# vsois/hanabi-agents

Hardware: AMD Instinct MI355X
Metric: env_steps_per_sec (higher is better)
Workload: dtype u8 env/encoder + bfloat16 Q-net GEMM (fp32 accumulate, fp32 master weights)

## Files before the change

hanabi-agents_amd/csrc/actor_fused.hip:

```cpp
#include <hip/hip_runtime.h>
#include <hip/hip_bf16.h>
#include <hip/hip_fp16.h>

#include <cstdint>
#include <type_traits>

#include "../../include/hanabi_hip.h"
#include "common.hpp"
#include "env_kernel.hpp"

using hb::fail;

namespace {

typedef __bf16 bf16x8 __attribute__((ext_vector_type(8)));
typedef _Float16 f16x8 __attribute__((ext_vector_type(8)));
typedef float f32x4 __attribute__((ext_vector_type(4)));

constexpr int FM = 128;
constexpr int FH = 512;
constexpr int FNT = 512;
constexpr int FK = 51;
constexpr int S2 = FH / 32;
constexpr int LUT_BYTES = 65536;
// ... 391 lines not shown
      if (ea < A && row < a.m) {
        const float* f = reinterpret_cast<const float*>(lds + H_BYTES) + (4 * g) * FM + rr;
        const float m0 = f[0], m1 = f[FM], m2 = f[2 * FM], m3 = f[3 * FM];
        const float M = fmaxf(fmaxf(m0, m1), fmaxf(m2, m3));
        const float e0 = exp2_fast(m0 - M), e1 = exp2_fast(m1 - M), e2 = exp2_fast(m2 - M), e3 = exp2_fast(m3 - M);
        const float* fs = f + 8 * FM;
        const float* ft = f + 16 * FM;
        const float S = fs[0] * e0 + fs[FM] * e1 + fs[2 * FM] * e2 + fs[3 * FM] * e3;
        const float T = ft[0] * e0 + ft[FM] * e1 + ft[2 * FM] * e2 + ft[3 * FM] * e3;
        a.q[row * A + ea] = T * __builtin_amdgcn_rcpf(S) * (1.0f / FK);
      }
    }
    if (p + 1 < n_pass) __syncthreads();
    if (p < 2) HB_FSTAMP(9 + 3 * p);
  }
  if (a.legal) {
    asm volatile("s_waitcnt vmcnt(0)" ::: "memory");
    __syncthreads();
    if (tid < FM && row0 + tid < a.m) {
      const long long g = row0 + tid;
      const unsigned long long gid = static_cast<unsigned long long>(a.first_gid + g);
      uint32_t rnd[4];
      hb::philox4x32_10(static_cast<uint32_t>(a.draw), static_cast<uint32_t>(a.draw >> 32), static_cast<uint32_t>(gid),
                        static_cast<uint32_t>(gid >> 32), static_cast<uint32_t>(a.seed), static_cast<uint32_t>(a.seed >> 32), rnd);
      const float* qr = a.q + g * A;
      const int8_t* lr = a.legal + g * A;
      float best = -INFINITY;
      unsigned long long legal_mask = 0, ties = 0;
      for (int i = 0; i < A; ++i) {
        const float v = __hip_atomic_load(qr + i, __ATOMIC_RELAXED, __HIP_MEMORY_SCOPE_AGENT);
        if (lr[i] != 0) {
          legal_mask |= 1ull << i;
          if (v > best) { best = v; ties = 1ull << i; }
          else if (v == best) ties |= 1ull << i;
        }
      }
      const float u = static_cast<float>(rnd[0] >> 8) * (1.0f / 16777216.0f);
      unsigned long long pool = (u < a.epsilon) ? legal_mask : ties;
      if (pool == 0) pool = legal_mask;
      int pick = 0;
      const int c = __popcll(pool);
      if (c > 0) {
        int k = static_cast<int>(__umulhi(rnd[1], static_cast<uint32_t>(c)));
        while (k-- > 0) pool &= pool - 1;
        pick = __ffsll(static_cast<long long>(pool)) - 1;
      }
      a.actions[g] = pick;
      if constexpr (!std::is_void_v<K>) reinterpret_cast<int*>(lds + H_BYTES)[tid] = pick;
    }
  }
  if constexpr (!std::is_void_v<K>) {
    constexpr int ENV_WORDS = hb::env_lds_words<K, EG>();
    static_assert((FM / EG) * ENV_WORDS * 4 <= H_BYTES && FM / EG <= FNT / 64, "env tail: the LDS slices must fit in H");
    __syncthreads();
    if (wave < FM / EG) {
#if defined(__HIP_DEVICE_COMPILE__)
      typedef const __attribute__((address_space(4))) unsigned char KargByte;
      typedef const __attribute__((address_space(4))) hb::EnvArgs KargEnv;
      auto kargs = __builtin_amdgcn_kernarg_segment_ptr();
      asm volatile("" : "+s"(kargs));
      constexpr size_t ENV_OFF = (sizeof(FusedArgs) + alignof(hb::EnvArgs) - 1) / alignof(hb::EnvArgs) * alignof(hb::EnvArgs);
      KargEnv& env = *(KargEnv*)((KargByte*)kargs + ENV_OFF);
#else
      const hb::EnvArgs env{};
#endif
      const long long g0 = row0 + EG * wave;
      const int uid = lane < EG ? reinterpret_cast<const int*>(lds + H_BYTES)[EG * wave + lane] : 0;
      hb::env_wave_step<K, EG>(env, g0, lane, reinterpret_cast<uint32_t*>(lds) + wave * ENV_WORDS, uid, g0 / EG);
    }
  }
  HB_FSTAMP_REAL(15);
}

template <bool F16>
__global__ __launch_bounds__(FNT) void actor_fused_kernel(const FusedArgs a) {
  actor_fused_body<F16, void, 16>(a);
}

template <bool F16, class K, int EG>
__global__ __launch_bounds__(FNT) void actor_env_fused_kernel(const FusedArgs a, const hb::EnvArgs env) {
  (void)env;
  actor_fused_body<F16, K, EG>(a);
}

template <bool F16>
__global__ __launch_bounds__(FNT) void actor_fused_grouped_kernel(const FusedArgs a, const hb_fused_tile* __restrict__ tiles) {
  const hb_fused_tile& t = tiles[blockIdx.x];
  if (!t.active) return;
  FusedArgs b = a;
  b.w1f = static_cast<const uint4*>(t.w1f); b.b1 = t.b1f; b.w2f = static_cast<const uint4*>(t.w2f); b.b2 = t.b2f;
  b.support = t.support;
  b.first_gid = t.first_game_id - static_cast<long long>(blockIdx.x) * FM;
  actor_fused_body<F16, void, 16>(b);
}

struct PackArgs {
  const __hip_bfloat16* w1; int w1_ld;
  const __hip_bfloat16* b1;
  const __hip_bfloat16* w2; int w2_ld;
  const __hip_bfloat16* b2;
  int obs_len, s1, n_actions, n_pass;
  uint4* w1f; float* b1f; uint4* w2f; float* b2f;
  int chunks1, chunks2;
  int f16;
  uint16_t* w1t; int w1t_ld;
  uint16_t* w2t; int w2t_ld;
};
__device__ __forceinline__ float bias_to_float(const __hip_bfloat16* b, int i, int f16) {
  return f16 ? __half2float(reinterpret_cast<const __half*>(b)[i]) : __bfloat162float(b[i]);
}
__host__ __device__ __forceinline__ int fused_logit(int col, int n_actions, int n_pass) {
  const int slot = col >> 6, c = col & 63, n = c >> 4, q = (c >> 2) & 3, j = c & 3;
  const int r16 = 4 * n + j;
  const int full_cap = 8 * n_pass;
  int action, atom;
  if (r16 < 12 || (r16 == 12 && q < 3)) {
    action = slot < full_cap ? slot : n_actions;
    if (action >= n_actions) return -1;
    atom = r16 < 12 ? 4 * r16 + q : 48 + q;
  } else {
    const int p = slot >> 3, w = slot & 7, f = w & 3;
// ... 280 lines not shown
```

hanabi-agents_amd/csrc/env_api.hip:

```cpp
#include <hip/hip_runtime.h>

#include <cstdarg>
#include <cstdio>
#include <cstdlib>
#include <cstring>
#include <new>
#include <string>
#include <vector>

#include "../../include/hanabi_hip.h"
#include "common.hpp"
#include "env_kernel.hpp"

namespace hb {
const EnvVariant* variants_full(int* n);
const EnvVariant* variants_small(int* n);
const EnvVariant* variants_vsmall(int* n);

thread_local std::string g_error;
int fail(int code, const char* fmt, ...) {
  char buf[512];
  va_list ap;
  va_start(ap, fmt);
  vsnprintf(buf, sizeof buf, fmt, ap);
  va_end(ap);
  g_error = buf;
  return code;
}

const EnvVariant* find_variant(const hb_config* c) {
  const EnvVariant* (*tables[])(int*) = {variants_full, variants_small, variants_vsmall};
  for (auto get : tables) {
    int n = 0;
    const EnvVariant* v = get(&n);
    for (int i = 0; i < n; ++i)
      if (v[i].P == c->players && v[i].C == c->colors && v[i].R == c->ranks && v[i].H == c->hand_size &&
          v[i].INFO == c->max_info && v[i].LIFE == c->max_life)
        return &v[i];
  }
  return nullptr;
}

static int copies_of(const hb_config* c, int r) { return r == 0 ? 3 : (r == c->ranks - 1 ? 1 : 2); }
static int deck_of(const hb_config* c) {
  int per = 0;
  for (int r = 0; r < c->ranks; ++r) per += copies_of(c, r);
  return per * c->colors;
}
}

struct hb_env {
  hb_config cfg;
  const hb::EnvVariant* var;
  long long n;
  unsigned long long seed;
  long long first_gid;
  uint32_t* state;
  unsigned long long* illegal;
  long long stat_slots;
  uint8_t* next_deck;
  uint8_t* refill;
  const uint8_t* decks;
  int gpw;
  int device;
  hipEvent_t ev_start, ev_stop;
  hipStream_t side;
  hipEvent_t ev_step_done, ev_refill_done;
  bool refill_in_flight;
  bool async_refill;
  int refill_period, since_refill;
  uint16_t* perms;
  uint8_t* shuf_mask;
  bool shuffled;
};

using hb::fail;

template <int C>
__global__ void color_perms_draw_kernel(const uint32_t* __restrict__ state, int sw, const uint8_t* __restrict__ mask, long long n, int P,
                                        unsigned long long seed, long long first_gid, uint16_t* __restrict__ perms) {
  const long long g = static_cast<long long>(blockIdx.x) * blockDim.x + threadIdx.x;
  if (g >= n) return;
  const uint32_t episode = state[g * sw + 6], m = mask[g];
  uint32_t e[hb::PERM_SLOTS / 2] = {0u, 0u, 0u, 0u};
  for (int p = 0; p < P; ++p) {
    const uint32_t sg = ((m >> p) & 1u) ? hb::draw_perm<C>(seed, static_cast<unsigned long long>(first_gid + g), episode, p)
                                        : hb::identity_perm(C);
    e[p >> 1] |= sg << (16 * (p & 1));
  }
  reinterpret_cast<uint4*>(perms)[g] = make_uint4(e[0], e[1], e[2], e[3]);
}

__global__ void color_perms_export_kernel(const uint16_t* __restrict__ perms, long long n, int P, int C, uint8_t* __restrict__ out) {
  const long long i = static_cast<long long>(blockIdx.x) * blockDim.x + threadIdx.x;
  if (i >= n * P * C) return;
  const long long g = i / (P * C);
  const int r = static_cast<int>(i - g * P * C), p = r / C, c = r - p * C;
  out[i] = static_cast<uint8_t>(perms ? (perms[g * hb::PERM_SLOTS + p] >> (3 * c)) & 7u : static_cast<uint32_t>(c));
}

__global__ void color_perms_import_kernel(const uint8_t* __restrict__ in, long long n, int P, int C, uint16_t* __restrict__ perms) {
  const long long g = static_cast<long long>(blockIdx.x) * blockDim.x + threadIdx.x;
  if (g >= n) return;
  uint32_t e[hb::PERM_SLOTS / 2] = {0u, 0u, 0u, 0u};
  for (int p = 0; p < P; ++p) {
    uint32_t sg = 0;
    for (int c = 0; c < C; ++c) sg |= static_cast<uint32_t>(in[(g * P + p) * C + c] & 7u) << (3 * c);
    e[p >> 1] |= sg << (16 * (p & 1));
  }
  reinterpret_cast<uint4*>(perms)[g] = make_uint4(e[0], e[1], e[2], e[3]);
}

static int draw_color_perms(hb_env* e, void* stream) {
  if (!e->shuffled) return HB_OK;
  const unsigned blocks = static_cast<unsigned>((e->n + 255) / 256);
  const hipStream_t st = static_cast<hipStream_t>(stream);
  const int P = e->cfg.players, sw = e->var->state_words;
  switch (e->cfg.colors) {
    case 1: hipLaunchKernelGGL(color_perms_draw_kernel<1>, dim3(blocks), dim3(256), 0, st, e->state, sw, e->shuf_mask, e->n, P, e->seed, e->first_gid, e->perms); break;
    case 2: hipLaunchKernelGGL(color_perms_draw_kernel<2>, dim3(blocks), dim3(256), 0, st, e->state, sw, e->shuf_mask, e->n, P, e->seed, e->first_gid, e->perms); break;
    case 3: hipLaunchKernelGGL(color_perms_draw_kernel<3>, dim3(blocks), dim3(256), 0, st, e->state, sw, e->shuf_mask, e->n, P, e->seed, e->first_gid, e->perms); break;
    case 4: hipLaunchKernelGGL(color_perms_draw_kernel<4>, dim3(blocks), dim3(256), 0, st, e->state, sw, e->shuf_mask, e->n, P, e->seed, e->first_gid, e->perms); break;
    default: hipLaunchKernelGGL(color_perms_draw_kernel<5>, dim3(blocks), dim3(256), 0, st, e->state, sw, e->shuf_mask, e->n, P, e->seed, e->first_gid, e->perms); break;
// ... 9 lines not shown

int hb_config_validate(const hb_config* c) {
  if (!c) return fail(HB_ERR_INVALID, "null config");
  if (c->players < 2 || c->players > 5) return fail(HB_ERR_INVALID, "players must be 2..5 (got %d)", c->players);
  if (c->colors < 1 || c->colors > 5) return fail(HB_ERR_INVALID, "colors must be 1..5 (got %d)", c->colors);
  if (c->ranks < 1 || c->ranks > 5) return fail(HB_ERR_INVALID, "ranks must be 1..5 (got %d)", c->ranks);
  if (c->hand_size < 1 || c->hand_size > 5) return fail(HB_ERR_INVALID, "hand_size must be 1..5 (got %d)", c->hand_size);
  if (c->max_info < 1 || c->max_info > 15) return fail(HB_ERR_INVALID, "max_info must be 1..15");
  if (c->max_life < 1 || c->max_life > 7) return fail(HB_ERR_INVALID, "max_life must be 1..7");
  if (c->players * c->hand_size > hb::deck_of(c)) return fail(HB_ERR_INVALID, "deck too small for the hands");
  return HB_OK;
}
int hb_num_actions(const hb_config* c) { return 2 * c->hand_size + (c->players - 1) * (c->colors + c->ranks); }
int hb_deck_size(const hb_config* c) { return hb::deck_of(c); }
int hb_obs_len(const hb_config* c) {
  const int bits = c->colors * c->ranks, P = c->players, H = c->hand_size, D = hb::deck_of(c);
  return (P - 1) * H * bits + P + (D - P * H + bits + c->max_info + c->max_life) + D +
         (P + 4 + P + c->colors + c->ranks + H + H + bits + 2) + P * H * (bits + c->colors + c->ranks);
}
int hb_state_words(const hb_config* c) { return c->players <= 3 ? 32 : 48; }
int hb_obs_words(const hb_config* c) { return (hb_obs_len(c) + 31) / 32; }

int hb_env_create(const hb_config* cfg, int64_t n_games, uint64_t seed, int64_t first_game_id, hb_env** out) {
  if (!out) return fail(HB_ERR_INVALID, "null out");
  *out = nullptr;
  if (int rc = hb_config_validate(cfg)) return rc;
  if (n_games <= 0) return fail(HB_ERR_INVALID, "n_games must be positive");
  const hb::EnvVariant* var = hb::find_variant(cfg);
  if (!var)
    return fail(HB_ERR_INVALID,
                "no compiled kernel for players=%d colors=%d ranks=%d hand=%d info=%d life=%d "
                "(built: Hanabi-Full / -Small / -Very-Small, 2..5 players)",
                cfg->players, cfg->colors, cfg->ranks, cfg->hand_size, cfg->max_info, cfg->max_life);
  if (var->obs_len != hb_obs_len(cfg) || var->n_actions != hb_num_actions(cfg) || var->deck != hb_deck_size(cfg))
    return fail(HB_ERR_INVALID, "internal: kernel sizes disagree with host formulas");
  int ndev = 0;
  if (hipGetDeviceCount(&ndev) != hipSuccess || ndev <= 0) return fail(HB_ERR_NO_DEVICE, "no HIP device available");
  hb_env* e = new (std::nothrow) hb_env();
  if (!e) return fail(HB_ERR_NOMEM, "out of host memory");
  e->cfg = *cfg;
  e->var = var;
  e->n = n_games;
  e->seed = seed;
  e->first_gid = first_game_id;
  e->decks = nullptr;
  e->gpw = 0;
  e->ev_start = e->ev_stop = nullptr;
  e->side = nullptr;
  e->ev_step_done = e->ev_refill_done = nullptr;
  e->refill_in_flight = false;
  e->async_refill = false;
  e->refill_period = cfg->max_life < 3 ? cfg->max_life : 3;
  e->since_refill = 0;
  e->perms = nullptr;
  e->shuf_mask = nullptr;
  e->shuffled = false;
  HB_HIP_OR(hipGetDevice(&e->device), delete e);
  const size_t bytes = static_cast<size_t>(n_games) * var->state_words * 4;
  HB_HIP_OR(hipMalloc(reinterpret_cast<void**>(&e->state), bytes), delete e);
  e->stat_slots = n_games / 8 + 8;
  HB_HIP_OR(hipMalloc(reinterpret_cast<void**>(&e->illegal), 8 + 16 * e->stat_slots), { (void)hipFree(e->state); delete e; });
  HB_HIP_OR(hipMemset(e->state, 0, bytes), { hb_env_destroy(e); });
  HB_HIP_OR(hipMemset(e->illegal, 0, 8 + 16 * e->stat_slots), { hb_env_destroy(e); });
  HB_HIP_OR(hipMalloc(reinterpret_cast<void**>(&e->next_deck), static_cast<size_t>(n_games) * hb::NEXT_DECK_BYTES), { hb_env_destroy(e); });
  HB_HIP_OR(hipMalloc(reinterpret_cast<void**>(&e->refill), static_cast<size_t>(n_games)), { hb_env_destroy(e); });
  HB_HIP_OR(hipMemset(e->next_deck, 0, static_cast<size_t>(n_games) * hb::NEXT_DECK_BYTES), { hb_env_destroy(e); });
  HB_HIP_OR(hipMemset(e->refill, 1, static_cast<size_t>(n_games)), { hb_env_destroy(e); });
  HB_HIP_OR(hipStreamCreateWithFlags(&e->side, hipStreamNonBlocking), { hb_env_destroy(e); });
  HB_HIP_OR(hipEventCreateWithFlags(&e->ev_step_done, hipEventDisableTiming), { hb_env_destroy(e); });
  HB_HIP_OR(hipEventCreateWithFlags(&e->ev_refill_done, hipEventDisableTiming), { hb_env_destroy(e); });
  *out = e;
  return HB_OK;
}

int hb_env_destroy(hb_env* e) {
  if (!e) return HB_OK;
  if (e->state) (void)hipFree(e->state);
  if (e->illegal) (void)hipFree(e->illegal);
  if (e->next_deck) (void)hipFree(e->next_deck);
  if (e->refill) (void)hipFree(e->refill);
  if (e->perms) (void)hipFree(e->perms);
  if (e->shuf_mask) (void)hipFree(e->shuf_mask);
  if (e->side) { (void)hipStreamSynchronize(e->side); (void)hipStreamDestroy(e->side); }
  if (e->ev_step_done) (void)hipEventDestroy(e->ev_step_done);
  if (e->ev_refill_done) (void)hipEventDestroy(e->ev_refill_done);
  delete e;
  return HB_OK;
}

int64_t hb_env_num_games(const hb_env* e) { return e ? e->n : 0; }

int hb_env_set_decks(hb_env* e, const uint8_t* decks_dev) {
  if (!e) return fail(HB_ERR_INVALID, "null env");
  e->decks = decks_dev;
  e->refill_in_flight = false;
  HB_HIP(hipDeviceSynchronize());
  HB_HIP(hipMemset(e->refill, 1, static_cast<size_t>(e->n)));
  return HB_OK;
}

int hb_env_set_games_per_wave(hb_env* e, int32_t g) {
  if (!e) return fail(HB_ERR_INVALID, "null env");
  if (g != 0 && g != 8 && g != 16 && g != 32 && g != 64)
    return fail(HB_ERR_INVALID, "games per wave must be 0 (automatic), 8, 16, 32 or 64");
  e->gpw = g;
  return HB_OK;
}

int hb_env_set_profile_events(hb_env* e, void* start_event, void* stop_event) {
  if (!e) return fail(HB_ERR_INVALID, "null env");
  if ((start_event == nullptr) != (stop_event == nullptr)) return fail(HB_ERR_INVALID, "pass both events or neither");
  e->ev_start = static_cast<hipEvent_t>(start_event);
  e->ev_stop = static_cast<hipEvent_t>(stop_event);
  return HB_OK;
}

static void fill_common(hb_env* e, hb::EnvArgs& a) {
  a.state = e->state;
  a.decks = e->decks;
  a.next_deck = e->next_deck;
  a.refill = e->refill;
  a.illegal = e->illegal;
  a.stats = e->illegal + 1;
  a.n = e->n;
  a.seed = e->seed;
  a.first_gid = e->first_gid;
  a.flags = e->cfg.flags;
}

static int join_refill(hb_env* e, void* stream) {
  if (e->refill_in_flight) {
    HB_HIP(hipStreamWaitEvent(static_cast<hipStream_t>(stream), e->ev_refill_done, 0));
    e->refill_in_flight = false;
  }
  return HB_OK;
}

static int refill(hb_env* e, void* stream) {
  e->since_refill = 0;
  hb::EnvArgs a{};
  fill_common(e, a);
  e->var->refill(a, static_cast<hipStream_t>(stream));
  HB_HIP(hipGetLastError());
  return HB_OK;
}

static int refill_async(hb_env* e, void* stream) {
  if (++e->since_refill < e->refill_period) return HB_OK;
  if (!e->async_refill) return refill(e, stream);
  HB_HIP(hipEventRecord(e->ev_step_done, static_cast<hipStream_t>(stream)));
  HB_HIP(hipStreamWaitEvent(e->side, e->ev_step_done, 0));
  if (int rc = refill(e, e->side)) return rc;
  HB_HIP(hipEventRecord(e->ev_refill_done, e->side));
  e->refill_in_flight = true;
  return HB_OK;
}

static void prepare(hb_env* e, hb::EnvArgs& a) {
  a.state = e->state;
  a.decks = e->decks;
  a.next_deck = e->next_deck;
  a.refill = e->refill;
  a.illegal = e->illegal;
  a.stats = e->illegal + 1;
  a.n = e->n;
  a.seed = e->seed;
  a.first_gid = e->first_gid;
  a.flags = e->cfg.flags;
  a.ev_start = e->ev_start;
  a.ev_stop = e->ev_stop;
  a.perms = e->shuffled ? e->perms : nullptr;
  a.shuf_mask = e->shuffled ? e->shuf_mask : nullptr;
}

static int launch(hb_env* e, hb::EnvArgs& a, void* stream) {
  prepare(e, a);
  const int gpw = e->gpw ? e->gpw : ((a.obs_bits && !a.obs && e->n >= 32768) ? 32 : 16);
  const hb::EnvVariant& v = *e->var;
  hb::LaunchFn fn = e->shuffled ? (gpw == 8 ? v.s8 : (gpw == 16 ? v.s16 : (gpw == 32 ? v.s32 : v.s64)))
                                : (gpw == 8 ? v.g8 : (gpw == 16 ? v.g16 : (gpw == 32 ? v.g32 : v.g64)));
  fn(a, static_cast<hipStream_t>(stream));
  HB_HIP(hipGetLastError());
  return HB_OK;
}

static int check_out(const void* obs, const void* legal) {
  if (!obs || !legal) return fail(HB_ERR_INVALID, "obs_dev and legal_dev are required");
  if ((reinterpret_cast<uintptr_t>(obs) & 15) || (reinterpret_cast<uintptr_t>(legal) & 15))
    return fail(HB_ERR_ALIGN, "obs_dev / legal_dev must be 16-byte aligned");
  return HB_OK;
}
static int check_out_packed(const void* bits, const void* obs, const void* legal) {
// ... 160 lines not shown
  if (!e) return fail(HB_ERR_INVALID, "null env");
  if (!q_dev || !sel_legal_dev || !actions_out_dev) return fail(HB_ERR_INVALID, "q_dev, sel_legal_dev and actions_out_dev are required");
  if ((reinterpret_cast<uintptr_t>(q_dev) & 15) || (reinterpret_cast<uintptr_t>(sel_legal_dev) & 3))
    return fail(HB_ERR_ALIGN, "q_dev must be 16-byte and sel_legal_dev 4-byte aligned");
  if (e->var->n_actions > 64) return fail(HB_ERR_INVALID, "the fused selection handles at most 64 actions");
  if (int rc = check_out_packed(obs_bits_dev, obs_dev, legal_dev)) return rc;
  hb::EnvArgs a{};
  a.mode = hb::MODE_STEP;
  a.sel_q = q_dev;
  a.sel_legal = sel_legal_dev;
  a.sel_actions = actions_out_dev;
  a.sel_eps = epsilon;
  a.sel_seed = seed;
  a.sel_draw = draw;
  a.sel_first_gid = first_game_id;
  a.obs = obs_dev;
  a.obs_bits = obs_bits_dev;
  a.legal = legal_dev;
  a.reward = reward_dev;
  a.terminal = terminal_dev;
  a.agent_reward = agent_reward_dev;
  a.agent_step_type = agent_step_type_dev;
  a.score = score_dev;
  if (int rc = join_refill(e, stream)) return rc;
  if (int rc = launch(e, a, stream)) return rc;
  return refill_async(e, stream);
}

int hb_actor_fused_act_step(hb_env* e, const uint32_t* obs_bits_dev, const int8_t* legal_dev, int64_t n_rows, int32_t obs_len,
                            const void* w1f_dev, const float* b1f_dev, const void* w2f_dev, const float* b2f_dev, const float* support_dev,
                            int32_t hidden, int32_t n_actions, int32_t n_atoms, float* q_dev, float epsilon, uint64_t seed, uint64_t draw,
                            int64_t first_game_id, int32_t* actions_dev, int32_t dtype, uint32_t* obs_bits_out_dev, int8_t* legal_out_dev,
                            float* reward_dev, int8_t* terminal_dev, float* agent_reward_dev, int8_t* agent_step_type_dev,
                            int8_t* score_dev, void* stream) {
  if (!e) return fail(HB_ERR_INVALID, "null env");
  if (e->shuffled) return fail(HB_ERR_INVALID, "the fused policy + env kernel has no colour-permuted form: step a shuffled env with "
                                               "hb_env_step_packed or hb_env_step_select_packed");
  if (int rc = check_out_packed(obs_bits_out_dev, nullptr, legal_out_dev)) return rc;
  hb::EnvArgs a{};
  a.mode = hb::MODE_STEP;
  a.obs_bits = obs_bits_out_dev;
  a.legal = legal_out_dev;
  a.reward = reward_dev;
  a.terminal = terminal_dev;
  a.agent_reward = agent_reward_dev;
  a.agent_step_type = agent_step_type_dev;
  a.score = score_dev;
  prepare(e, a);
  if (int rc = join_refill(e, stream)) return rc;
  if (int rc = hb::actor_env_fused_launch(obs_bits_dev, legal_dev, n_rows, obs_len, w1f_dev, b1f_dev, w2f_dev, b2f_dev, support_dev, hidden,
                                          n_actions, n_atoms, q_dev, epsilon, seed, draw, first_game_id, actions_dev, dtype, a, *e->var,
                                          stream))
    return rc;
  return refill_async(e, stream);
}

int hb_actor_fused_step_supported(const hb_env* e) { return e && !e->shuffled && hb::actor_env_fused_supported(*e->var) ? 1 : 0; }

#ifdef HB_STAMPS
int hb_env_step_stamped(hb_env* e, const int32_t* actions_dev, int8_t* obs_dev, int8_t* legal_dev,
                        unsigned long long* stamps_dev, void* stream) {
  hb::EnvArgs a{};
  a.mode = hb::MODE_STEP;
  a.actions = actions_dev;
  a.obs = obs_dev;
  a.legal = legal_dev;
  a.stamps = stamps_dev;
  if (int rc = join_refill(e, stream)) return rc;
  if (int rc = launch(e, a, stream)) return rc;
  return refill_async(e, stream);
}
#endif

int hb_env_illegal_count(hb_env* e, int64_t* out) {
  if (!e || !out) return fail(HB_ERR_INVALID, "null argument");
  unsigned long long v = 0;
  HB_HIP(hipMemcpy(&v, e->illegal, 8, hipMemcpyDeviceToHost));
  *out = static_cast<int64_t>(v);
  return HB_OK;
}

int hb_env_stats(hb_env* e, int64_t* episodes, int64_t* score_sum) {
  if (!e || !episodes || !score_sum) return fail(HB_ERR_INVALID, "null argument");
  std::vector<unsigned long long> v(static_cast<size_t>(2 * e->stat_slots));
  HB_HIP(hipMemcpy(v.data(), e->illegal + 1, 16 * e->stat_slots, hipMemcpyDeviceToHost));
  unsigned long long ep = 0, sc = 0;
  for (long long i = 0; i < e->stat_slots; ++i) { ep += v[2 * i]; sc += v[2 * i + 1]; }
  *episodes = static_cast<int64_t>(ep);
  *score_sum = static_cast<int64_t>(sc);
  return HB_OK;
}

int hb_env_set_refill_period(hb_env* e, int32_t steps) {
  if (!e) return fail(HB_ERR_INVALID, "null env");
  if (steps < 1 || steps > e->cfg.max_life) return fail(HB_ERR_INVALID, "refill period must be 1..max_life (%d)", e->cfg.max_life);
  e->refill_period = steps;
  return HB_OK;
}

int hb_env_set_async_refill(hb_env* e, int32_t on) {
  if (!e) return fail(HB_ERR_INVALID, "null env");
  HB_HIP(hipDeviceSynchronize());
  e->refill_in_flight = false;
  e->async_refill = on != 0;
  return HB_OK;
}

// ... 77 lines not shown
```

hanabi-agents_amd/csrc/env_kernel.hpp:

```cpp
#pragma once
#include <hip/hip_runtime.h>
#include <hip/hip_ext.h>
#include <stdint.h>
#include <utility>

struct hb_config;

namespace hb {

enum { MODE_STEP = 0, MODE_OBSERVE = 1, MODE_RESET = 2 };
constexpr int NEXT_DECK_BYTES = 64;
enum { MV_PLAY = 0, MV_DISCARD = 1, MV_RCOLOR = 2, MV_RRANK = 3 };

struct EnvArgs {
  uint32_t* state;
  const int32_t* actions;
  const uint8_t* mask;
  const uint8_t* decks;
  uint8_t* next_deck;
  uint8_t* refill;
  int8_t* obs;
  uint32_t* obs_bits;
  int8_t* legal;
  float* reward;
// ... 356 lines not shown
      dv |= ((disc >> (c * K::CPC)) & ((1ull << K::CPC) - 1ull)) << (K::CPC * sig(c));
    });
    acc.template put64<K::DISC_OFF, K::D>(dv);
  } else {
    acc.template put64<K::DISC_OFF, K::D>(disc);
  }
  {
    const uint32_t valid = w2 & 1u;
    const int la_player = (w2 >> 1) & 7, la_type = (w2 >> 4) & 3, la_ci = (w2 >> 6) & 7, la_toff = (w2 >> 9) & 7;
    const int la_color_t = (w2 >> 12) & 7, la_rank = (w2 >> 15) & 7;
    const int la_color = SHUF ? sig(la_color_t) : la_color_t;
    const uint32_t la_scored = (w2 >> 18) & 1u, la_info = (w2 >> 19) & 1u, la_mask = (w2 >> 20) & 31u;
    int actor = la_player - o;
    if (actor < 0) actor += P;
    int target = actor + la_toff;
    if (target >= P) target -= P;
    const uint32_t reveal = valid & static_cast<uint32_t>(la_type >= MV_RCOLOR);
    const uint32_t cardmv = valid & static_cast<uint32_t>(la_type <= MV_DISCARD);
    const uint32_t is_rc = valid & static_cast<uint32_t>(la_type == MV_RCOLOR);
    const uint32_t is_rr = valid & static_cast<uint32_t>(la_type == MV_RRANK);
    const uint32_t is_play = valid & static_cast<uint32_t>(la_type == MV_PLAY);
    constexpr int o1 = K::LA_OFF, o2 = o1 + P, o3 = o2 + 4, o4 = o3 + P, o5 = o4 + C, o6 = o5 + R, o7 = o6 + H,
                  o8 = o7 + H, o9 = o8 + K::BITS;
    acc.template put<o1, P>(valid << actor);
    acc.template put<o2, 4>(valid << la_type);
    acc.template put<o3, P>(reveal << target);
    acc.template put<o4, C>(is_rc << la_color);
    acc.template put<o5, R>(is_rr << la_rank);
    acc.template put<o6, H>(reveal ? la_mask : 0u);
    acc.template put<o7, H>(cardmv << la_ci);
    acc.template put<o8, K::BITS>(cardmv << (la_color * R + la_rank));
    acc.template put<o9, 2>((is_play & la_scored) | ((is_play & la_info) << 1));
  }
  static_for<P>([&](auto REL) {
    constexpr int rel = decltype(REL)::value;
    int p = o + rel;
    if (p >= P) p -= P;
    const int n_p = hand_n(p);
    const uint64_t kn = (static_cast<uint64_t>(row[K::W_KNOW + 2 * p + 1]) << 32) | row[K::W_KNOW + 2 * p];
    static_for<H>([&](auto I) {
      constexpr int i = decltype(I)::value;
      const uint32_t k = static_cast<uint32_t>(kn >> (12 * i)) & 0xFFFu;
      const uint32_t cp = seen_colours<SHUF, C>(k & 31u, sg), rp = (k >> 5) & 31u;
      const uint32_t plaus = __umul24(spread_colors<C, R>(cp), rp);
      const uint32_t ch = (k >> 10) & 1u, rh = (k >> 11) & 1u;
      uint64_t v = plaus | (static_cast<uint64_t>(ch ? cp : 0u) << K::BITS) |
                   (static_cast<uint64_t>(rh ? rp : 0u) << (K::BITS + C));
      if (i >= n_p) v = 0;
      acc.template put64<K::KN_OFF + (rel * H + i) * K::KN_SLOT, K::KN_SLOT>(v);
    });
  });
}

template <class K, int G, bool SHUF = false>
__device__ __forceinline__ void env_wave_step(const EnvArgs& a, long long g0, int lane, uint32_t* const srow, int uid_in,
                                              long long wslot) {
  constexpr int P = K::P, C = K::C, R = K::R, H = K::H;
  constexpr int LPG = 1;
  uint32_t* const obits = srow + G * K::SWP;
  uint32_t* const lbits = obits + G * K::NWP;
  const long long left = a.n - g0;
  const int nvalid = left <= 0 ? 0 : (left < G ? static_cast<int>(left) : G);
  const int mode = a.mode;
  HB_STAMP_REAL(10);
  HB_STAMP(0);

  const bool active = lane < nvalid && lane < G;
  const long long gi = g0 + lane;
  bool mask_in = true;
  uint4 nd[4] = {make_uint4(0u, 0u, 0u, 0u), make_uint4(0u, 0u, 0u, 0u), make_uint4(0u, 0u, 0u, 0u), make_uint4(0u, 0u, 0u, 0u)};
  const uint4* const ndp = reinterpret_cast<const uint4*>(a.next_deck + gi * NEXT_DECK_BYTES);
  if (active) {
    if (mode == MODE_RESET && a.mask) mask_in = a.mask[gi] != 0;
    if (mode == MODE_RESET && mask_in) {
      nd[0] = ndp[0]; nd[1] = ndp[1]; nd[2] = ndp[2]; nd[3] = ndp[3];
    }
  }
  uint4 pm = make_uint4(0u, 0u, 0u, 0u);
  if constexpr (SHUF) {
    if (active) pm = reinterpret_cast<const uint4*>(a.perms)[gi];
  }

  {
    constexpr int Q = K::SW / 4;
    constexpr int ROUNDS = (G * Q + 63) / 64;
    const uint4* src = reinterpret_cast<const uint4*>(a.state + g0 * K::SW);
    uint4 v[ROUNDS];
#pragma unroll
    for (int r = 0; r < ROUNDS; ++r) {
      const int e = lane + 64 * r;
      v[r] = e < nvalid * Q ? src[e] : make_uint4(0u, 0u, 0u, 0u);
    }
#pragma unroll
    for (int r = 0; r < ROUNDS; ++r) {
      const int e = lane + 64 * r;
      if (e < nvalid * Q) {
        const int g = e / Q, q = e - g * Q;
        uint32_t* d = srow + g * K::SWP + 4 * q;
        d[0] = v[r].x; d[1] = v[r].y; d[2] = v[r].z; d[3] = v[r].w;
      }
    }
  }
  HB_STAMP(1);
  wave_sync();
  HB_STAMP(2);

  uint32_t* const row = srow + lane * K::SWP;
  uint32_t w0 = 0, w1 = 0, w2 = 0, w3 = 0, w6 = 0;
  uint64_t accw = 0, disc = 0;
// ... 111 lines not shown
        if (success) w1 += 1u << (3 * c_col);
        {
          const int dpos = (c_col * K::CPC + (c_rank ? 2 * c_rank + 1 : 0)) & 63;
          const uint32_t dmask = c_rank == 0 ? 7u : (c_rank == R - 1 ? 1u : 3u);
          const uint32_t dfield = static_cast<uint32_t>(disc >> dpos) & dmask;
          const uint32_t dnew = to_discard ? (((dfield << 1) | 1u) & dmask) : 0u;
          disc |= static_cast<uint64_t>(dnew) << dpos;
        }
        const int info2 = info + (card_move ? la_info : -1);
        const int life2 = life - (fail ? 1 : 0);
        const int deck2 = deck_size - ((card_move && draws) ? 1 : 0);
        const int turns2 = turns - (deck_size == 0 ? 1 : 0);
        const int la_color = card_move ? c_col : hcol, la_rank = card_move ? c_rank : hrank;
        w2 = 1u | (static_cast<uint32_t>(s) << 1) | (static_cast<uint32_t>(type) << 4) | (static_cast<uint32_t>(ci) << 6) |
             (static_cast<uint32_t>(toff) << 9) | (static_cast<uint32_t>(la_color) << 12) |
             (static_cast<uint32_t>(la_rank) << 15) | (static_cast<uint32_t>(success ? 1 : 0) << 18) |
             (static_cast<uint32_t>(card_move ? la_info : 0) << 19) | (match << 20);
        int cur = s + 1;
        if (cur >= P) cur = 0;
        w0 = static_cast<uint32_t>(deck2) | (static_cast<uint32_t>(info2) << 6) | (static_cast<uint32_t>(life2) << 10) |
             (static_cast<uint32_t>(cur) << 13) | (static_cast<uint32_t>(turns2 & 7) << 16) |
             (static_cast<uint32_t>((moves + 1) & 255) << 21);
        const int after = score_now();
        int status = 0;
        if (life2 < 1) status = 1;
        else if (after >= C * R) status = 2;
        else if (turns2 <= 0) status = 3;
        w0 |= static_cast<uint32_t>(status) << 19;
        int r = after - before;
        if ((a.flags & 4) && r < 0) r = 0;
        out_reward = static_cast<float>(r);
        out_term = status != 0;
#pragma unroll
        for (int q = 0; q < P; ++q) {
          const bool live = ((w3 >> q) & 1u) && !((w3 >> (5 + q)) & 1u);
          const int8_t v = static_cast<int8_t>(static_cast<int8_t>(accw >> (8 * q)) + (live ? r : 0));
          accw = (accw & ~(0xFFull << (8 * q))) | (static_cast<uint64_t>(static_cast<uint8_t>(v)) << (8 * q));
          if (live && out_term) w3 |= 1u << (5 + q);
        }
        if (out_term && (a.flags & 1)) {
          need_reset = true;
          reset_start = (a.flags & 2) ? cur : 0;
        }
      }
    }
    out_score = score_now();
  }

  HB_STAMP(3);
  if (active && need_reset) {
    const uint32_t* ndw = reinterpret_cast<const uint32_t*>(nd);
#pragma unroll
    for (int i = 0; i < 13; ++i) row[K::W_DECK + i] = ndw[i];
    a.refill[gi] = 1;
  }
  HB_STAMP(4);
  wave_sync();
  HB_STAMP(5);

  if (active) {
    if (need_reset) {
      const uint8_t* deckb = reinterpret_cast<const uint8_t*>(row + K::W_DECK);
      w0 = static_cast<uint32_t>(K::D - P * H) | (static_cast<uint32_t>(K::INFO) << 6) | (static_cast<uint32_t>(K::LIFE) << 10) |
           (static_cast<uint32_t>(reset_start) << 13) | (static_cast<uint32_t>(P) << 16);
      w1 = 0;
      w2 = 0;
      if (!keep_seats) { w3 = 0; accw = 0; }
      w6 += 1;
      disc = 0;
#pragma unroll
      for (int p = 0; p < P; ++p) {
        uint32_t hc = 0;
        uint64_t kn = 0;
#pragma unroll
        for (int i = 0; i < 5; ++i) {
          if (i < H) {
            hc |= static_cast<uint32_t>(deckb[p * H + i]) << (5 * i);
            kn |= static_cast<uint64_t>(K::ALL_PLAUSIBLE) << (12 * i);
          } else {
            hc |= 31u << (5 * i);
          }
        }
        row[K::W_HANDS + p] = hc;
        row[K::W_KNOW + 2 * p] = static_cast<uint32_t>(kn);
        row[K::W_KNOW + 2 * p + 1] = static_cast<uint32_t>(kn >> 32);
        w1 |= static_cast<uint32_t>(H) << (15 + 3 * p);
      }
      if constexpr (SHUF) {
        const uint32_t sm = a.shuf_mask[gi];
        uint32_t e[PERM_SLOTS / 2] = {0u, 0u, 0u, 0u};
#pragma unroll
        for (int p = 0; p < P; ++p) {
          const uint32_t sg = ((sm >> p) & 1u) ? draw_perm<C>(a.seed, static_cast<unsigned long long>(a.first_gid + gi), w6, p)
                                               : identity_perm(C);
          e[p >> 1] |= sg << (16 * (p & 1));
        }
        pm = make_uint4(e[0], e[1], e[2], e[3]);
        reinterpret_cast<uint4*>(a.perms)[gi] = pm;
      }
    }
    if (mode != MODE_OBSERVE) {
      row[0] = w0; row[1] = w1; row[2] = w2; row[3] = w3;
      row[4] = static_cast<uint32_t>(accw); row[5] = static_cast<uint32_t>(accw >> 32);
      row[6] = w6; row[7] = 0;
      row[8] = static_cast<uint32_t>(disc); row[9] = static_cast<uint32_t>(disc >> 32);
    }

// ... 18 lines not shown
      }
      const uint32_t pend = (w3 >> o) & 1u, tsin = (w3 >> (5 + o)) & 1u;
      if (a.agent_reward) a.agent_reward[gi] = pend ? static_cast<float>(static_cast<int8_t>(accw >> (8 * o))) : 0.f;
      if (a.agent_step_type) a.agent_step_type[gi] = static_cast<int8_t>(!pend ? 0 : (tsin ? 2 : 1));
      if (mode == MODE_STEP) {
        if (a.reward) a.reward[gi] = out_reward;
        if (a.terminal) a.terminal[gi] = static_cast<int8_t>(out_term);
        if (a.score) a.score[gi] = static_cast<int8_t>(out_score);
      }
    }
  }
  if (mode == MODE_STEP) {
    const unsigned long long bad = __ballot(illegal);
    if (bad && lane == 0) atomicAdd(a.illegal, static_cast<unsigned long long>(__popcll(bad)));
    const unsigned long long ended = __ballot(out_term != 0);
    if (ended) {
      int sc = out_term ? out_score : 0;
      for (int o = 32; o > 0; o >>= 1) sc += __shfl_xor(sc, o);
      if (lane == 0) {
        unsigned long long* slot = a.stats + 2 * wslot;
        atomicAdd(slot, static_cast<unsigned long long>(__popcll(ended)));
        atomicAdd(slot + 1, static_cast<unsigned long long>(sc));
      }
    }
  }
  HB_STAMP(6);
  wave_sync();
  HB_STAMP(7);

  if (mode != MODE_OBSERVE) {
    constexpr int Q = K::SW / 4;
    uint4* dst = reinterpret_cast<uint4*>(a.state + g0 * K::SW);
    for (int e = lane; e < nvalid * Q; e += 64) {
      const int g = e / Q, q = e - g * Q;
      const uint32_t* s = srow + g * K::SWP + 4 * q;
      uint4 v;
      v.x = s[0]; v.y = s[1]; v.z = s[2]; v.w = s[3];
      dst[e] = v;
    }
  }
  HB_STAMP(8);
  if (mode != MODE_RESET) {
    if (a.obs_bits) {
      uint32_t* dst = a.obs_bits + g0 * K::NW;
      for (int e = lane; e < nvalid * K::NW; e += 64) {
        const int g = e / K::NW, i = e - g * K::NW;
        dst[e] = obits[g * K::NWP + i];
      }
    }
    if (a.obs) expand_rows<K::OBS_LEN>(obits, K::NWP, nvalid, a.obs + g0 * K::OBS_LEN, lane);
    expand_rows<K::A>(lbits, K::LW, nvalid, a.legal + g0 * K::A, lane);
  }
  HB_STAMP(9);
  HB_STAMP_REAL(11);
}

template <class K, int G>
__global__ __launch_bounds__(256) void env_kernel(const EnvArgs a) {
  __shared__ uint32_t lds[4 * env_lds_words<K, G>()];
  const int lane = threadIdx.x & 63;
  const int wave = threadIdx.x >> 6;
  const long long wslot = static_cast<long long>(blockIdx.x) * 4 + wave;
  const long long g0 = wslot * G;
  int uid_in = 0;
  if (a.mode == MODE_STEP && lane < G && g0 + lane < a.n) uid_in = a.sel_q ? select_action<K::A>(a, g0 + lane) : a.actions[g0 + lane];
  env_wave_step<K, G>(a, g0, lane, lds + wave * env_lds_words<K, G>(), uid_in, wslot);
}

template <class K, int G>
__global__ __launch_bounds__(256) void env_kernel_shuf(const EnvArgs a) {
  __shared__ uint32_t lds[4 * env_lds_words<K, G>()];
  const int lane = threadIdx.x & 63;
  const int wave = threadIdx.x >> 6;
  const long long wslot = static_cast<long long>(blockIdx.x) * 4 + wave;
  const long long g0 = wslot * G;
  int uid_in = 0;
  if (a.mode == MODE_STEP && lane < G && g0 + lane < a.n) uid_in = a.sel_q ? select_action<K::A>(a, g0 + lane) : a.actions[g0 + lane];
  env_wave_step<K, G, true>(a, g0, lane, lds + wave * env_lds_words<K, G>(), uid_in, wslot);
}

template <class K>
__global__ __launch_bounds__(256) void refill_kernel(const EnvArgs a) {
  constexpr int GR = 16;
  const int lane = threadIdx.x & 63;
  const long long g0 = (static_cast<long long>(blockIdx.x) * 4 + (threadIdx.x >> 6)) * GR;
  if (g0 >= a.n) return;
  const long long gi = g0 + lane;
  const bool mine = lane < GR && gi < a.n && a.refill[gi] != 0;
  unsigned long long todo = __ballot(mine);
  while (todo) {
    const int src = __ffsll(static_cast<long long>(todo)) - 1;
    todo &= todo - 1;
    const long long g = g0 + src;
    uint8_t* dst = a.next_deck + g * NEXT_DECK_BYTES;
    if (a.decks) {
      if (lane < K::D) dst[lane] = a.decks[g * K::D + lane];
    } else {
      const uint32_t episode = a.state[g * K::SW + 6];
      const unsigned long long gid = static_cast<unsigned long long>(a.first_gid + g);
      uint32_t out[4];
      philox4x32_10(static_cast<uint32_t>(lane), episode, static_cast<uint32_t>(gid), static_cast<uint32_t>(gid >> 32),
                    static_cast<uint32_t>(a.seed), static_cast<uint32_t>(a.seed >> 32), out);
      const uint32_t key = (out[0] & ~63u) | static_cast<uint32_t>(lane);
      int rank = 0;
      static_for<K::D>([&](auto I) {
        constexpr int i = decltype(I)::value;
        const uint32_t ki = static_cast<uint32_t>(__builtin_amdgcn_readlane(static_cast<int>(key), i));
        rank += ki < key ? 1 : 0;
      });
      if (lane < K::D) {
        const int col = lane / K::CPC, k = lane - col * K::CPC;
        const int rk = k < 3 ? 0 : 1 + (k - 3) / 2;
        dst[rank] = static_cast<uint8_t>(col * K::R + rk);
      }
    }
  }
  if (mine) a.refill[gi] = 0;
}

template <class K>
void launch_refill(const EnvArgs& a, hipStream_t stream) {
  const unsigned blocks = static_cast<unsigned>((a.n + 63) / 64);
  if (blocks == 0) return;
  hipLaunchKernelGGL((refill_kernel<K>), dim3(blocks), dim3(256), 0, stream, a);
}

template <class K, int G>
void launch_env(const EnvArgs& a, hipStream_t stream) {
  const long long per_block = 4LL * G;
  const unsigned blocks = static_cast<unsigned>((a.n + per_block - 1) / per_block);
  if (blocks == 0) return;
  if (a.ev_start && a.ev_stop)
    hipExtLaunchKernelGGL((env_kernel<K, G>), dim3(blocks), dim3(256), 0, stream, a.ev_start, a.ev_stop, 0, a);
  else
    hipLaunchKernelGGL((env_kernel<K, G>), dim3(blocks), dim3(256), 0, stream, a);
}

template <class K, int G>
void launch_env_shuf(const EnvArgs& a, hipStream_t stream) {
  const long long per_block = 4LL * G;
  const unsigned blocks = static_cast<unsigned>((a.n + per_block - 1) / per_block);
  if (blocks == 0) return;
  if (a.ev_start && a.ev_stop)
    hipExtLaunchKernelGGL((env_kernel_shuf<K, G>), dim3(blocks), dim3(256), 0, stream, a.ev_start, a.ev_stop, 0, a);
  else
    hipLaunchKernelGGL((env_kernel_shuf<K, G>), dim3(blocks), dim3(256), 0, stream, a);
}

struct EncodeArgs {
  const uint32_t* rows;
  uint32_t* obs_bits;
  int8_t* obs;
  int8_t* legal;
  long long n;
  int seat;
};

template <class K, int G>
__global__ __launch_bounds__(256) void encode_rows_kernel(const EncodeArgs a) {
  __shared__ uint32_t lds[4 * env_lds_words<K, G>()];
  const int lane = threadIdx.x & 63;
  const int wave = threadIdx.x >> 6;
  const long long g0 = (static_cast<long long>(blockIdx.x) * 4 + wave) * G;
  uint32_t* const srow = lds + wave * env_lds_words<K, G>();
  uint32_t* const obits = srow + G * K::SWP;
  uint32_t* const lbits = obits + G * K::NWP;
  const long long left = a.n - g0;
// ... 93 lines not shown
```

Before: 314.7 million.

## Regenerate next decks inside fused actor-env kernel instead of separate refill launch

The fused actor+env kernel now collects the games that reset this step, shares them across wavefronts through LDS after a block barrier, and has the wavefronts regenerate those games' next decks in round-robin order. The refill flag is no longer set, and the host skips the async refill kernel when no refill is pending. This removes a separate kernel launch and the side-stream synchronisation per step. In exchange it adds a block-wide barrier and deck shuffling to the tail of the fused kernel, which may unbalance wavefronts.

```diff
diff --git a/hanabi-agents_amd/csrc/actor_fused.hip b/hanabi-agents_amd/csrc/actor_fused.hip
--- a/hanabi-agents_amd/csrc/actor_fused.hip
+++ b/hanabi-agents_amd/csrc/actor_fused.hip
@@ -467,6 +467,8 @@
   if constexpr (!std::is_void_v<K>) {
     constexpr int ENV_WORDS = hb::env_lds_words<K, EG>();
     static_assert((FM / EG) * ENV_WORDS * 4 <= H_BYTES && FM / EG <= FNT / 64, "env tail: the LDS slices must fit in H");
+    static_assert(FM / EG == FNT / 64 && (FM / EG & (FM / EG - 1)) == 0 && EG <= 32 && ENV_WORDS > EG,
+                  "env tail: every wavefront steps games and meets the others at the barrier before the pool rows are regenerated");
     __syncthreads();
     if (wave < FM / EG) {
 #if defined(__HIP_DEVICE_COMPILE__)
@@ -481,7 +483,24 @@
 #endif
       const long long g0 = row0 + EG * wave;
       const int uid = lane < EG ? reinterpret_cast<const int*>(lds + H_BYTES)[EG * wave + lane] : 0;
-      hb::env_wave_step<K, EG>(env, g0, lane, reinterpret_cast<uint32_t*>(lds) + wave * ENV_WORDS, uid, g0 / EG);
+      uint32_t* const slice = reinterpret_cast<uint32_t*>(lds) + wave * ENV_WORDS;
+      hb::Redeals rd;
+      hb::env_wave_step<K, EG, false, true>(env, g0, lane, slice, uid, g0 / EG, &rd);
+      if (lane == 0) slice[0] = static_cast<uint32_t>(rd.lanes);
+      if (lane < EG) slice[1 + lane] = rd.deal;
+      __syncthreads();
+      int r = 0;
+      for (int v = 0; v < FM / EG; ++v) {
+        const uint32_t* const sv = reinterpret_cast<const uint32_t*>(lds) + v * ENV_WORDS;
+        uint32_t todo = __builtin_amdgcn_readfirstlane(sv[0]);
+        while (todo) {
+          const int src = __ffs(todo) - 1;
+          todo &= todo - 1;
+          if ((r++ & (FM / EG - 1)) != wave) continue;
+          const long long g = row0 + EG * v + src;
+          hb::shuffle_deck<K>(env, g, __builtin_amdgcn_readfirstlane(sv[1 + src]), env.next_deck + g * hb::NEXT_DECK_BYTES, lane);
+        }
+      }
     }
   }
   HB_FSTAMP_REAL(15);
diff --git a/hanabi-agents_amd/csrc/env_api.hip b/hanabi-agents_amd/csrc/env_api.hip
--- a/hanabi-agents_amd/csrc/env_api.hip
+++ b/hanabi-agents_amd/csrc/env_api.hip
@@ -69,6 +69,7 @@
   bool refill_in_flight;
   bool async_refill;
   int refill_period, since_refill;
+  bool pool_stale;
   uint16_t* perms;
   uint8_t* shuf_mask;
   bool shuffled;
@@ -184,6 +185,7 @@
   e->async_refill = false;
   e->refill_period = cfg->max_life < 3 ? cfg->max_life : 3;
   e->since_refill = 0;
+  e->pool_stale = true;
   e->perms = nullptr;
   e->shuf_mask = nullptr;
   e->shuffled = false;
@@ -228,6 +230,7 @@
   e->refill_in_flight = false;
   HB_HIP(hipDeviceSynchronize());
   HB_HIP(hipMemset(e->refill, 1, static_cast<size_t>(e->n)));
+  e->pool_stale = true;
   return HB_OK;
 }
 
@@ -270,6 +273,7 @@
 
 static int refill(hb_env* e, void* stream) {
   e->since_refill = 0;
+  e->pool_stale = false;
   hb::EnvArgs a{};
   fill_common(e, a);
   e->var->refill(a, static_cast<hipStream_t>(stream));
@@ -536,7 +540,8 @@
                                           n_actions, n_atoms, q_dev, epsilon, seed, draw, first_game_id, actions_dev, dtype, a, *e->var,
                                           stream))
     return rc;
-  return refill_async(e, stream);
+  if (e->since_refill > 0 || e->pool_stale) return refill_async(e, stream);
+  return HB_OK;
 }
 
 int hb_actor_fused_step_supported(const hb_env* e) { return e && !e->shuffled && hb::actor_env_fused_supported(*e->var) ? 1 : 0; }
diff --git a/hanabi-agents_amd/csrc/env_kernel.hpp b/hanabi-agents_amd/csrc/env_kernel.hpp
--- a/hanabi-agents_amd/csrc/env_kernel.hpp
+++ b/hanabi-agents_amd/csrc/env_kernel.hpp
@@ -432,9 +432,33 @@
   });
 }
 
-template <class K, int G, bool SHUF = false>
+template <class K>
+__device__ __forceinline__ void shuffle_deck(const EnvArgs& a, long long g, uint32_t episode, uint8_t* dst, int lane) {
+  const unsigned long long gid = static_cast<unsigned long long>(a.first_gid + g);
+  uint32_t out[4];
+  philox4x32_10(static_cast<uint32_t>(lane), episode, static_cast<uint32_t>(gid), static_cast<uint32_t>(gid >> 32),
+                static_cast<uint32_t>(a.seed), static_cast<uint32_t>(a.seed >> 32), out);
+  const uint32_t key = (out[0] & ~63u) | static_cast<uint32_t>(lane);
+  int rank = 0;
+  static_for<K::D>([&](auto I) {
+    constexpr int i = decltype(I)::value;
+    const uint32_t ki = static_cast<uint32_t>(__builtin_amdgcn_readlane(static_cast<int>(key), i));
+    rank += ki < key ? 1 : 0;
+  });
+  if (lane < K::D) {
+    const int col = lane / K::CPC, k = lane - col * K::CPC;
+    const int rk = k < 3 ? 0 : 1 + (k - 3) / 2;
+    dst[rank] = static_cast<uint8_t>(col * K::R + rk);
+  }
+}
+
+struct Redeals {
+  unsigned long long lanes;
+  uint32_t deal;
+};
+template <class K, int G, bool SHUF = false, bool REGEN = false>
 __device__ __forceinline__ void env_wave_step(const EnvArgs& a, long long g0, int lane, uint32_t* const srow, int uid_in,
-                                              long long wslot) {
+                                              long long wslot, Redeals* rd = nullptr) {
   constexpr int P = K::P, C = K::C, R = K::R, H = K::H;
   constexpr int LPG = 1;
   uint32_t* const obits = srow + G * K::SWP;
@@ -652,7 +676,7 @@
     const uint32_t* ndw = reinterpret_cast<const uint32_t*>(nd);
 #pragma unroll
     for (int i = 0; i < 13; ++i) row[K::W_DECK + i] = ndw[i];
-    a.refill[gi] = 1;
+    if constexpr (!REGEN) a.refill[gi] = 1;
   }
   HB_STAMP(4);
   wave_sync();
@@ -777,6 +801,10 @@
     expand_rows<K::A>(lbits, K::LW, nvalid, a.legal + g0 * K::A, lane);
   }
   HB_STAMP(9);
+  if constexpr (REGEN) {
+    rd->lanes = mode == MODE_STEP && a.decks == nullptr ? __ballot(active && need_reset) : 0ull;
+    rd->deal = w6;
+  }
   HB_STAMP_REAL(11);
 }
 
@@ -822,22 +850,7 @@
       if (lane < K::D) dst[lane] = a.decks[g * K::D + lane];
     } else {
       const uint32_t episode = a.state[g * K::SW + 6];
-      const unsigned long long gid = static_cast<unsigned long long>(a.first_gid + g);
-      uint32_t out[4];
-      philox4x32_10(static_cast<uint32_t>(lane), episode, static_cast<uint32_t>(gid), static_cast<uint32_t>(gid >> 32),
-                    static_cast<uint32_t>(a.seed), static_cast<uint32_t>(a.seed >> 32), out);
-      const uint32_t key = (out[0] & ~63u) | static_cast<uint32_t>(lane);
-      int rank = 0;
-      static_for<K::D>([&](auto I) {
-        constexpr int i = decltype(I)::value;
-        const uint32_t ki = static_cast<uint32_t>(__builtin_amdgcn_readlane(static_cast<int>(key), i));
-        rank += ki < key ? 1 : 0;
-      });
-      if (lane < K::D) {
-        const int col = lane / K::CPC, k = lane - col * K::CPC;
-        const int rk = k < 3 ? 0 : 1 + (k - 3) / 2;
-        dst[rank] = static_cast<uint8_t>(col * K::R + rk);
-      }
+      shuffle_deck<K>(a, g, episode, dst, lane);
     }
   }
   if (mine) a.refill[gi] = 0;
```

New measurement: 312.6 million. No clear change (-0.7%).
